# alibaba/pairec

Hardware: AMD Instinct MI355X
Metric: ranked items/sec, 5k-cand DNN rank (recall top-5000 of 100M x 128 -> DNN3 -> fuse -> sort) (higher is better)
Workload: dtype bf16x3; 1 GPU; configs[1]+[2]: recall 5k of 100000000x128 fp32 table in HBM -> 3-layer DNN rank (256-512-256-1, bf16 MFMA with split hi + lo operands = bf16x3, fp32-accurate scores) -> RankScore fusion (fp64) -> ItemRankScore sort; candidates_per_request=5000, table_rows=100000000, dim=128, table_dist=uniform, batches_in_flight=2, contexts=2, all_batches_on_predicted_thresholds=True, batches_re_run_after_a_failed_plan=0, parallelism=1 GPU

## Files before the change

### pairec_amd/csrc/common.hpp

```cpp
#pragma once
#include <hip/hip_runtime.h>

#include <algorithm>
#include <cstdarg>
#include <cstdint>
#include <cstdio>
#include <cstring>
#include <map>
#include <atomic>
#include <memory>
#include <mutex>
#include <shared_mutex>
#include <string>
#include <vector>

#include "../../include/pairec_gpu.h"

namespace pg {

struct PipeRun;
void set_error(const char* fmt, ...);

#define PG_HIP(expr)                                                                           \
    do {                                                                                       \
// ... 404 lines not shown
int rescreen16_prep_launch(pg_ctx* ctx, const pg_table* t, const RecallScratch& rs, uint32_t nq);
int rescreen16_launch(pg_ctx* ctx, const pg_table* t, const RecallScratch& rs, uint32_t nq);
int screen4m_launch(pg_ctx* ctx, const pg_table* t, const RecallScratch& rs, uint32_t nq, uint32_t row_begin, uint32_t row_end,
                    uint32_t cap1, bool susp2_clean = false);
int topk_merge_strided_locked(pg_ctx* ctx, const uint64_t* d_rows, const float* d_scores, uint32_t nq, uint32_t nlists,
                              uint32_t per_list, size_t row_ls, size_t row_qs, size_t sc_ls, size_t sc_qs, uint32_t k,
                              uint64_t* d_out_rows, float* d_out_scores, uint32_t* d_out_count);
int topk_merge_locked(pg_ctx* ctx, const uint64_t* d_rows, const float* d_scores, uint32_t nq, uint32_t nlists,
                      uint32_t per_list, int list_major, uint32_t k, uint64_t* d_out_rows, float* d_out_scores,
                      uint32_t* d_out_count);

int rank_dnn3_dev_locked(pg_ctx* ctx, const pg_model* m, const pg_table* t, const float* d_user,
                         const uint32_t* d_cand, const uint32_t* d_off, uint32_t n_req, uint32_t n_items,
                         float* d_out, size_t out_stride = 0);
int fm2t_user_embedding_locked(pg_ctx* ctx, const pg_model* m, const float* d_user, uint32_t n_req, float* d_out);
int rank_fm2t_irows_dev_locked(pg_ctx* ctx, const pg_model* m, const pg_item_rows* ir, const float* d_user, const int32_t* d_ufids,
                               const uint32_t* d_cand, const uint32_t* d_off, uint32_t n_req, uint32_t n_items, float* d_out);
int rank_fm2t_rows_dev_locked(pg_ctx* ctx, const pg_model* m, const pg_features* fs, const int32_t* item_field_cols,
                              const float* d_user, const int32_t* d_ufids, const uint32_t* d_cand, const uint32_t* d_off,
                              uint32_t n_req, uint32_t n_items, float* d_out);
int expr_eval_enqueue_locked(pg_ctx* ctx, const pg_expr* e, const double* d_vars, uint32_t n_items, double* d_out,
                             uint32_t* d_err, uint32_t items_per_flag);
void set_expr_arith_error(const pg_expr* e);
constexpr int kMaxRewrites = 8;
void expr_hold(const pg_expr* e);
void expr_release(const pg_expr* e);
struct ExprHold {
    const pg_expr* e = nullptr;
    ExprHold() = default;
    ExprHold(const ExprHold&) = delete;
    ExprHold& operator=(const ExprHold&) = delete;
    void take(const pg_expr* x) {
        if (e) expr_release(e);
        e = x;
        if (e) expr_hold(e);
    }
    ~ExprHold() { if (e) expr_release(e); }
};
int expr_num_rewrites(const pg_expr* e);
const char* expr_rewrite_source(const pg_expr* e, int r);
int expr_rewrite_num_vars(const pg_expr* e, int r);
const char* expr_rewrite_var_name(const pg_expr* e, int r, int i);
int expr_rewrite_eval_enqueue_locked(pg_ctx* ctx, const pg_expr* e, int r, const double* d_vars, uint32_t n_items, double* d_out,
                                     uint32_t* d_err, uint32_t items_per_flag);
int table_gather_locked(pg_ctx* ctx, const pg_table* t, const uint32_t* d_rows, uint32_t n, float* d_out);
int dpp_run_locked(pg_ctx* ctx, const float* d_emb32, const double* d_hook, const double* d_rel, uint32_t R, uint32_t n,
// ... 40 lines not shown
```

### pairec_amd/csrc/expr.hip

```cpp
#include "common.hpp"

#include <cmath>
#include <string>
#include <vector>

namespace pg {

enum OpCode : uint32_t { OP_CONST = 0, OP_VAR, OP_ADD, OP_SUB, OP_MUL, OP_DIV, OP_MOD, OP_POW, OP_FNZ,
                         OP_DIVF,
                         OP_NEG };

struct Instr {
    uint32_t op;
    uint32_t arg;
    double val;
};

constexpr int kMaxStack = 32;
constexpr int kMaxProg = 128;

}

struct pg_expr {
    std::string source;
// ... 243 lines not shown
            }
            if (i & 1) {
                a1 *= x1;
                ae += xe;
            }
            x1 *= x1;
            xe <<= 1;
            if (x1 < 0.5) {
                x1 += x1;
                xe--;
            }
        }
        if (y < 0.0) {
            a1 = 1.0 / a1;
            ae = -ae;
        }
        if (ae > 4096) ae = 4096;
        if (ae < -4096) ae = -4096;
        return ldexp(a1, (int)ae);
    }
    return pow(x, y);
}

__global__ void expr_eval_kernel(ExprDev e, const double* __restrict__ vars, uint32_t n_items,
                                 double* __restrict__ out, uint32_t* __restrict__ err, uint32_t items_per_flag) {
    const uint32_t i = blockIdx.x * blockDim.x + threadIdx.x;
    if (i >= n_items) return;
    double st[kMaxStack];
    int sp = 0;
    bool bad = false;
    for (uint32_t pc = 0; pc < e.n; ++pc) {
        const Instr in = e.prog[pc];
        if (in.op == OP_CONST) {
            st[sp++] = in.val;
        } else if (in.op == OP_VAR) {
            st[sp++] = vars[(size_t)in.arg * n_items + i];
        } else {
            if (in.op == OP_NEG) {
                st[sp - 1] = -st[sp - 1];
                continue;
            }
            const double r = st[--sp];
            const double l = st[--sp];
            double v = 0.0;
            switch (in.op) {
                case OP_DIVF: v = l / r; break;
                case OP_ADD: v = l + r; break;
                case OP_SUB: v = l - r; break;
                case OP_MUL: v = l * r; break;
                case OP_DIV:
                    if (r == 0.0) bad = true; else v = l / r;
                    break;
                case OP_MOD: {
                    const long long li = (l == l && fabs(l) < 9223372036854775808.0) ? (long long)l : (long long)0x8000000000000000ull;
                    const long long ri = (r == r && fabs(r) < 9223372036854775808.0) ? (long long)r : (long long)0x8000000000000000ull;
                    if (ri == 0) bad = true;
                    else if (ri == -1) v = 0.0;
                    else v = (double)(li % ri);
                    break;
                }
                case OP_POW: v = go_pow(l, r); break;
                case OP_FNZ: v = (l != 0.0) ? l : r; break;
            }
            st[sp++] = v;
        }
    }
    out[i] = sp > 0 ? st[sp - 1] : 0.0;
    if (bad) atomicOr(err + (items_per_flag ? i / items_per_flag : 0u), 1u);
}

int expr_eval_enqueue_locked(pg_ctx* ctx, const pg_expr* e, const double* d_vars, uint32_t n_items, double* d_out,
                             uint32_t* d_err, uint32_t items_per_flag) {
    if (e->empty) {
        PG_HIP(hipMemsetAsync(d_out, 0, (size_t)n_items * 8, ctx->stream));
    } else {
        ExprDev dev;
        dev.n = (uint32_t)e->prog.size();
        for (size_t i = 0; i < e->prog.size(); ++i) dev.prog[i] = e->prog[i];
        expr_eval_kernel<<<(n_items + 255) / 256, 256, 0, ctx->stream>>>(dev, d_vars, n_items, d_out, d_err, items_per_flag);
        PG_HIP(hipGetLastError());
    }
    return PG_OK;
}

int expr_num_rewrites(const pg_expr* e) { return e ? (int)e->rewrites.size() : 0; }
const char* expr_rewrite_source(const pg_expr* e, int r) { return e->rewrites[(size_t)r].source.c_str(); }
int expr_rewrite_num_vars(const pg_expr* e, int r) { return (int)e->rewrites[(size_t)r].vars.size(); }
const char* expr_rewrite_var_name(const pg_expr* e, int r, int i) { return e->rewrites[(size_t)r].vars[(size_t)i].c_str(); }
int expr_rewrite_eval_enqueue_locked(pg_ctx* ctx, const pg_expr* e, int r, const double* d_vars, uint32_t n_items, double* d_out,
                                     uint32_t* d_err, uint32_t items_per_flag) {
    const pg_expr::Rewrite& rw = e->rewrites[(size_t)r];
    if (rw.failed || rw.prog.empty()) {
        PG_HIP(hipMemsetAsync(d_out, 0, (size_t)n_items * 8, ctx->stream));
        return PG_OK;
    }
    ExprDev dev;
    dev.n = (uint32_t)rw.prog.size();
    for (size_t i = 0; i < rw.prog.size(); ++i) dev.prog[i] = rw.prog[i];
    expr_eval_kernel<<<(n_items + 255) / 256, 256, 0, ctx->stream>>>(dev, d_vars, n_items, d_out, d_err, items_per_flag);
    PG_HIP(hipGetLastError());
    return PG_OK;
}

void set_expr_arith_error(const pg_expr* e) {
    set_error("pg_expr_eval: violation of arithmetic specification: a division by zero in '%s' "
              "(the reference panics in ExprASTResult, utils/ast/ast.go:243-249)", e->source.c_str());
}

static int expr_eval_locked(pg_ctx* ctx, const pg_expr* e, const double* d_vars, uint32_t n_items,
                            double* d_out) {
    void* p;
    int rc;
    if ((rc = scratch_reserve(ctx, 4, 4096, &p))) return rc;
    uint32_t* d_err = (uint32_t*)p + 320;
    PG_HIP(hipMemsetAsync(d_err, 0, 4, ctx->stream));
    if ((rc = expr_eval_enqueue_locked(ctx, e, d_vars, n_items, d_out, d_err, 0))) return rc;
    PG_HIP(hipMemcpyAsync(ctx->h_status + 320, d_err, 4, hipMemcpyDeviceToHost, ctx->stream));
    PG_HIP(hipStreamSynchronize(ctx->stream));
    if (ctx->h_status[320] != 0) {
        set_expr_arith_error(e);
        return PG_ERR_ARITH;
    }
// ... 363 lines not shown
```

### pairec_amd/csrc/misc.hip

```cpp
#include "pipeline.hpp"

#include <algorithm>
#include <cstring>
#include <vector>

namespace pg {

__global__ void rows_to_local_kernel(const uint64_t* __restrict__ rows, uint32_t n, uint64_t off,
                                     uint64_t nrows, uint32_t* __restrict__ local,
                                     uint8_t* __restrict__ owned, uint32_t* __restrict__ uni_off, uint32_t uni_nq, uint32_t uni_k) {
    const uint32_t i = blockIdx.x * blockDim.x + threadIdx.x;
    if (uni_off && i <= uni_nq) uni_off[i] = i * uni_k;
    if (i >= n) return;
    const uint64_t r = rows[i];
    const bool mine = r != ~0ull && r >= off && r - off < nrows;
    local[i] = mine ? (uint32_t)(r - off) : 0u;
    if (owned) owned[i] = mine ? 1 : 0;
}

__global__ void widen_kernel(const float* __restrict__ in, uint32_t n, double* __restrict__ out) {
    const uint32_t i = blockIdx.x * blockDim.x + threadIdx.x;
    if (i < n) out[i] = (double)in[i];
}

typedef uint32_t u32x4 __attribute__((ext_vector_type(4)));
__global__ __launch_bounds__(256) void hbm_probe_kernel(const u32x4* __restrict__ p, uint64_t n16,
                                                        uint32_t* __restrict__ sink) {
    uint32_t acc = 0;
    const uint64_t stride = (uint64_t)gridDim.x * blockDim.x;
    uint64_t i = (uint64_t)blockIdx.x * blockDim.x + threadIdx.x;
    for (; i + 3 * stride < n16; i += 4 * stride) {
        const u32x4 a = __builtin_nontemporal_load(&p[i]);
        const u32x4 b = __builtin_nontemporal_load(&p[i + stride]);
        const u32x4 c = __builtin_nontemporal_load(&p[i + 2 * stride]);
        const u32x4 d = __builtin_nontemporal_load(&p[i + 3 * stride]);
// ... 79 lines not shown
                const uint64_t* d_rows, const float* d_recall, const float* d_rank, size_t rank_stride, int n_algos,
                const double* d_fused, uint32_t nq, uint32_t k, uint32_t top_n, char* d_page) {
    const size_t np = (size_t)nq * top_n;
    if (np == 0) return PG_OK;
    uint64_t* p_rows = (uint64_t*)d_page;
    double* p_fused = (double*)(p_rows + np);
    float* p_recall = (float*)(p_fused + np);
    float* p_rank = p_recall + np;
    page_kernel<<<(uint32_t)((np + 255) / 256), 256, 0, st>>>(d_order, d_pick, d_pick_cnt, d_rows, d_recall, d_rank, rank_stride, n_algos,
                                                             d_fused, nq, k, top_n, p_rows, p_fused, p_recall, p_rank);
    PG_HIP(hipGetLastError());
    return PG_OK;
}

int rows_to_local_locked(pg_ctx* ctx, const pg_table* t, const uint64_t* d_rows, uint32_t n, uint32_t* d_local,
                         uint8_t* d_owned) {
    if (n == 0) return PG_OK;
    rows_to_local_kernel<<<(n + 255) / 256, 256, 0, ctx->stream>>>(d_rows, n, t->row_offset, t->rows, d_local, d_owned, nullptr, 0, 0);
    PG_HIP(hipGetLastError());
    return PG_OK;
}

int rows_to_local_offsets_locked(pg_ctx* ctx, const pg_table* t, const uint64_t* d_rows, uint32_t nq, uint32_t k, uint32_t* d_local,
                                 uint32_t* d_off) {
    const uint32_t n = nq * k;
    if (n <= nq) {
        int rc = uniform_offsets_locked(ctx, nq, k, d_off);
        return rc ? rc : rows_to_local_locked(ctx, t, d_rows, n, d_local, nullptr);
    }
    rows_to_local_kernel<<<(n + 255) / 256, 256, 0, ctx->stream>>>(d_rows, n, t->row_offset, t->rows, d_local, nullptr, d_off, nq, k);
    PG_HIP(hipGetLastError());
    return PG_OK;
}

int uniform_offsets_locked(pg_ctx* ctx, uint32_t nq, uint32_t k, uint32_t* d_off) {
    uniform_offsets_kernel<<<(nq + 256) / 256, 256, 0, ctx->stream>>>(nq, k, d_off);
    PG_HIP(hipGetLastError());
    return PG_OK;
}

}

extern "C" {

int pg_hbm_read_probe(pg_ctx* ctx, const pg_table* t, int reps, double* out_gbps) {
    PG_REQUIRE(ctx && t && out_gbps && reps > 0, "pg_hbm_read_probe: bad argument");
    const void* d_buf = t->d;
    const uint64_t bytes = t->rows * (uint64_t)t->dim * 4;
    PG_REQUIRE(bytes >= (1u << 20), "pg_hbm_read_probe: table smaller than 1 MiB");
    std::lock_guard<std::mutex> g(ctx->mu);
    void* sink;
    int rc;
    if ((rc = pg::scratch_reserve(ctx, 4, 4096, &sink))) return rc;
// ... 37 lines not shown
```

### pairec_amd/csrc/pipeline.hip

```cpp
#include "pipeline.hpp"

#include <algorithm>
#include <chrono>
#include <thread>

namespace pg {

struct VarSrc { int8_t src[32]; };
__global__ void bind_vars_kernel(const float* __restrict__ recall, const float* __restrict__ rank, size_t rank_stride,
                                 uint32_t n, uint32_t nv, VarSrc vs, double* __restrict__ vars, uint32_t* __restrict__ err,
                                 const double* __restrict__ rw, int zero_err) {
    const uint32_t i = blockIdx.x * blockDim.x + threadIdx.x;
    if (zero_err && i < (uint32_t)kMaxQueries) err[i] = 0;
    if (i >= n) return;
    const double a = (double)recall[i];
    for (uint32_t v = 0; v < nv; ++v) {
        const int sa = vs.src[v];
        vars[(size_t)v * n + i] = sa >= 0 ? (double)rank[(size_t)sa * rank_stride + i] : (sa == -1 ? a : rw[(size_t)(-2 - sa) * n + i]);
    }
}

__global__ void mask_pads_kernel(const uint64_t* __restrict__ rows, uint32_t n, float* __restrict__ rank, size_t rank_stride,
                                 int n_algos, double* __restrict__ fused) {
    const uint32_t i = blockIdx.x * blockDim.x + threadIdx.x;
    if (i >= n || rows[i] != ~0ull) return;
    for (int a = 0; a < n_algos; ++a) rank[(size_t)a * rank_stride + i] = 0.0f;
    fused[i] = __longlong_as_double(0x7FF8000000000000ll);
}

int pipe_run_acquire(pg_ctx* ctx, PipeRun** out) {
    {
        std::lock_guard<std::mutex> g(ctx->pool_mu);
        if (!ctx->pipe_free.empty()) {
            *out = ctx->pipe_free.back();
            ctx->pipe_free.pop_back();
            return PG_OK;
        }
    }
    PG_HIP(hipSetDevice(ctx->device));
    PipeRun* r = new PipeRun();
    if (hipHostMalloc((void**)&r->h_status, kPipeStatusWords * 4) != hipSuccess || hipEventCreate(&r->done) != hipSuccess) {
        set_error("pipeline: cannot allocate a batch's status block: %s", hipGetErrorString(hipGetLastError()));
        if (r->h_status) hipHostFree(r->h_status);
// ... 74 lines not shown
    int wide = std::max(c.nv, 1);
    const int n_rw = expr_num_rewrites(c.e);
    for (int r = 0; r < n_rw; ++r) wide = std::max(wide, expr_rewrite_num_vars(c.e, r));
    const size_t b_vars = al((size_t)(wide + n_rw) * n * 8);
    if ((rc = scratch_reserve(ctx, 8, b_local + b_off + b_err + b_vars, &buf))) return rc;
    ps->d_local = (uint32_t*)buf;
    ps->d_off = (uint32_t*)((char*)buf + b_local);
    ps->d_err = (uint32_t*)((char*)buf + b_local + b_off);
    ps->d_vars = (double*)((char*)buf + b_local + b_off + b_err);
    ps->c_rows = nullptr; ps->c_rel = nullptr; ps->c_emb = nullptr; ps->c_bail = nullptr;
    if (c.rerank.kind) {
        const size_t nc = (size_t)nq * c.rerank.candidates;
        const size_t b_rows = al(nc * 8), b_rel = al(nc * 8), b_emb = al(nc * c.t->dim * 4), b_bail = al((size_t)kMaxQueries * 4);
        if ((rc = scratch_reserve(ctx, 10, b_rows + b_rel + b_emb + b_bail, &buf))) return rc;
        ps->c_rows = (uint64_t*)buf;
        ps->c_rel = (double*)((char*)buf + b_rows);
        ps->c_emb = (float*)((char*)buf + b_rows + b_rel);
        ps->c_bail = (uint32_t*)((char*)buf + b_rows + b_rel + b_emb);
    }
    return PG_OK;
}

int fuse_scores_enqueue_locked(pg_ctx* ctx, const pg_expr* e, const int* var_src, int nv, const float* d_recall, const float* d_rank,
                               size_t rank_stride, uint32_t n, uint32_t items_per_flag, double* d_vars, uint32_t* d_err, double* d_fused) {
    hipStream_t st = ctx->stream;
    int rc;
    VarSrc vs;
    const int n_rw = expr_num_rewrites(e);
    int wide = std::max(nv, 1);
    for (int r = 0; r < n_rw; ++r) wide = std::max(wide, expr_rewrite_num_vars(e, r));
    double* const d_rw = d_vars + (size_t)wide * n;
    const uint32_t bind_grid = (std::max(n, (uint32_t)kMaxQueries) + 255) / 256;
    bool zeroed = false;
    for (int r = 0, at = nv; r < n_rw; ++r) {
        const int nvr = expr_rewrite_num_vars(e, r);
        for (int i = 0; i < 32; ++i) vs.src[i] = i < nvr ? (int8_t)var_src[at + i] : (int8_t)-1;
        at += nvr;
        if (nvr > 0 || !zeroed) {
            bind_vars_kernel<<<bind_grid, 256, 0, st>>>(d_recall, d_rank, rank_stride, n, (uint32_t)nvr, vs, d_vars, d_err, nullptr, zeroed ? 0 : 1);
            PG_HIP(hipGetLastError());
            zeroed = true;
        }
        if ((rc = expr_rewrite_eval_enqueue_locked(ctx, e, r, d_vars, n, d_rw + (size_t)r * n, d_err, items_per_flag))) return rc;
    }
    for (int i = 0; i < 32; ++i) vs.src[i] = i < nv ? (int8_t)var_src[i] : (int8_t)-1;
    if (nv > 0) {
        bind_vars_kernel<<<bind_grid, 256, 0, st>>>(d_recall, d_rank, rank_stride, n, (uint32_t)nv, vs, d_vars, d_err, d_rw, zeroed ? 0 : 1);
        PG_HIP(hipGetLastError());
    } else if (!zeroed) {
        PG_HIP(hipMemsetAsync(d_err, 0, (size_t)kMaxQueries * 4, st));
    }
    return expr_eval_enqueue_locked(ctx, e, d_vars, n, d_fused, d_err, items_per_flag);
}

int post_fuse_sort_locked(pg_ctx* ctx, const RecommendCall& c, uint32_t q0, uint32_t nq, const PostScratch& ps) {
    const uint32_t n = nq * c.k;
    const size_t o = (size_t)q0 * c.k;
    hipStream_t st = ctx->stream;
    int rc;
    if ((rc = fuse_scores_enqueue_locked(ctx, c.e, c.var_src, c.nv, c.d_recall + o, c.d_rank + o, c.rank_stride, n, c.k, ps.d_vars, ps.d_err,
                                         c.d_fused + o)))
        return rc;
    if (c.pads) {
        mask_pads_kernel<<<(n + 255) / 256, 256, 0, st>>>(c.d_rows + o, n, c.d_rank + o, c.rank_stride, c.planes(), c.d_fused + o);
        PG_HIP(hipGetLastError());
    }
    return sort_dev_locked(ctx, c.d_fused + o, ps.d_off, nq, n, c.k, 1, c.d_order + o);
}

int rerank_select_locked(pg_ctx* ctx, const RecommendCall& c, uint32_t q0, uint32_t nq, const PostScratch& ps) {
    const uint32_t C = c.rerank.candidates;
    const size_t o = (size_t)q0 * c.k;
    if (c.k < C) {
        set_error("recommend: the DPP stage wants %u candidates, the lists hold k = %u", C, c.k);
        return PG_ERR_UNSUPPORTED;
    }
    int rc;
    if ((rc = sorted_head_launch(ctx->stream, c.d_order + o, c.d_rows + o, c.d_fused + o, nq, c.k, C, ps.c_rows, ps.c_rel))) return rc;
    return dpp_norm_relevance_launch(ctx->stream, ps.c_rel, nq, C, c.rerank.dpp.norm_relevance_score, ps.c_bail);
}
int rerank_run_locked(pg_ctx* ctx, const RecommendCall& c, uint32_t q0, uint32_t nq, const PostScratch& ps) {
    const uint32_t C = c.rerank.candidates;
    int rc;
    if ((rc = dpp_run_locked(ctx, ps.c_emb, nullptr, ps.c_rel, nq, C, c.t->dim, 0, c.rerank.dpp.alpha, c.top_n, c.rerank.dpp.window,
                             c.rerank.dpp.normalize_emb, 1, 1, c.d_pick + (size_t)q0 * c.top_n, c.d_pick_cnt + q0)))
        return rc;
    if (c.rerank.dpp.norm_relevance_score)
        return dpp_bail_fix_launch(ctx->stream, ps.c_bail, nq, C, c.top_n, c.d_pick + (size_t)q0 * c.top_n, c.d_pick_cnt + q0);
    return PG_OK;
}

static int recommend_post_locked(pg_ctx* ctx, const RecommendCall& c, uint32_t q0, uint32_t nq, const PostScratch& ps) {
    const uint32_t n = nq * c.k;
    const size_t o = (size_t)q0 * c.k;
    int rc;
    if ((rc = rows_to_local_offsets_locked(ctx, c.t, c.d_rows + o, nq, c.k, ps.d_local, ps.d_off))) return rc;
    for (int a = 0; a < c.n_algos; ++a) {
        const RankAlgoRef& al = c.algos[a];
        float* out = c.d_rank + (size_t)c.plane0[a] * c.rank_stride + o;
        const float* users = c.d_queries + (size_t)q0 * c.t->dim;
        if ((rc = rank_algo_locked(ctx, al, c.t, users, c.d_ufids ? c.d_ufids + (size_t)q0 * c.ufid_stride : nullptr, ps.d_local, ps.d_off, nq, n,
                                   out, c.rank_stride)))
            return rc;
    }
    if ((rc = post_fuse_sort_locked(ctx, c, q0, nq, ps))) return rc;
    if (c.rerank.kind == 1) {
        if (c.t->rows < c.rerank.candidates) {
            set_error("recommend: the DPP stage wants %u candidates, the table has %llu rows", c.rerank.candidates, (unsigned long long)c.t->rows);
            return PG_ERR_UNSUPPORTED;
        }
        if ((rc = rerank_select_locked(ctx, c, q0, nq, ps))) return rc;
        if ((rc = gather_global_rows_launch(ctx->stream, c.t, ps.c_rows, nq * c.rerank.candidates, ps.c_emb))) return rc;
        if ((rc = rerank_run_locked(ctx, c, q0, nq, ps))) return rc;
    }
    return PG_OK;
}

int rank_algo_locked(pg_ctx* ctx, const RankAlgoRef& al, const pg_table* t, const float* d_user, const int32_t* d_ufids,
                     const uint32_t* d_cand, const uint32_t* d_off, uint32_t n_req, uint32_t n_items, float* d_out, size_t out_stride) {
    if (al.m->kind == PG_MODEL_DNN3) return rank_dnn3_dev_locked(ctx, al.m, t, d_user, d_cand, d_off, n_req, n_items, d_out, out_stride);
    if (al.irows) return rank_fm2t_irows_dev_locked(ctx, al.m, al.irows, d_user, d_ufids, d_cand, d_off, n_req, n_items, d_out);
    return rank_fm2t_rows_dev_locked(ctx, al.m, al.fs, al.item_field_cols, d_user, d_ufids, d_cand, d_off, n_req, n_items, d_out);
}

int recommend_enqueue(pg_ctx* ctx, const RecommendCall& c, PipeRun* r, bool first) {
    if (c.t->d_row_map) {
        set_error("recommend: the table is a filtered view (pg_table_view_create) — views serve the recall calls only");
        return PG_ERR_UNSUPPORTED;
// ... 195 lines not shown
```

### pairec_amd/csrc/pipeline.hpp

```cpp
#pragma once
#include "common.hpp"

namespace pg {

struct RecommendCall;
struct PipeRun {
    RecallJob job;
    uint32_t* h_status = nullptr;
    std::vector<hipEvent_t> events;
    hipEvent_t done = nullptr;
    bool patched = false;
};
constexpr uint32_t kExprFlagAt = 320;
constexpr uint32_t kPipeStatusWords = 640;

int pipe_run_acquire(pg_ctx* ctx, PipeRun** out);
void pipe_run_release(pg_ctx* ctx, PipeRun* r);

constexpr int kMaxAlgos = 4;
struct RankAlgoRef {
    const pg_model* m = nullptr;
    const pg_features* fs = nullptr;
    int32_t item_field_cols[16] = {0};
    const pg_item_rows* irows = nullptr;
// ... 28 lines not shown
    int n_planes = 0;
    int planes() const { return n_planes ? n_planes : n_algos; }
    double* d_fused = nullptr;
    uint32_t* d_order = nullptr;
    uint32_t* d_count = nullptr;
    bool pads = false;
    RerankStage rerank;
    uint32_t top_n = 0;
    uint32_t* d_pick = nullptr;
    uint32_t* d_pick_cnt = nullptr;
};
int recommend_bind_vars(const pg_expr* e, const char* const* names, int n_algos, std::vector<int>* var_src, const char* who);
int recommend_enqueue(pg_ctx* ctx, const RecommendCall& c, PipeRun* r, bool first);
int recommend_verify(pg_ctx* ctx, PipeRun* r, bool* ok, const RecommendCall* c = nullptr);
struct PostScratch {
    uint32_t *d_local, *d_off, *d_err;
    double* d_vars;
    uint64_t* c_rows;
    double* c_rel;
    float* c_emb;
    uint32_t* c_bail;
};
int post_scratch(pg_ctx* ctx, const RecommendCall& c, uint32_t nq, PostScratch* ps);
int post_fuse_sort_locked(pg_ctx* ctx, const RecommendCall& c, uint32_t q0, uint32_t nq, const PostScratch& ps);
int fuse_scores_enqueue_locked(pg_ctx* ctx, const pg_expr* e, const int* var_src, int nv, const float* d_recall, const float* d_rank,
                               size_t rank_stride, uint32_t n, uint32_t items_per_flag, double* d_vars, uint32_t* d_err, double* d_fused);
int rerank_select_locked(pg_ctx* ctx, const RecommendCall& c, uint32_t q0, uint32_t nq, const PostScratch& ps);
int rerank_run_locked(pg_ctx* ctx, const RecommendCall& c, uint32_t q0, uint32_t nq, const PostScratch& ps);

int rows_to_local_locked(pg_ctx* ctx, const pg_table* t, const uint64_t* d_rows, uint32_t n, uint32_t* d_local,
                         uint8_t* d_owned);
int uniform_offsets_locked(pg_ctx* ctx, uint32_t nq, uint32_t k, uint32_t* d_off);
int rows_to_local_offsets_locked(pg_ctx* ctx, const pg_table* t, const uint64_t* d_rows, uint32_t nq, uint32_t k, uint32_t* d_local,
                                 uint32_t* d_off);
int sorted_head_launch(hipStream_t st, const uint32_t* d_order, const uint64_t* d_rows, const double* d_fused, uint32_t nq,
                       uint32_t k, uint32_t C, uint64_t* d_c_rows, double* d_c_rel);
int gather_global_rows_launch(hipStream_t st, const pg_table* t, const uint64_t* d_global_rows, uint32_t n, float* d_out);
size_t page_entry_bytes(int n_algos);
int page_launch(hipStream_t st, const uint32_t* d_order, const uint32_t* d_pick, const uint32_t* d_pick_cnt,
                const uint64_t* d_rows, const float* d_recall, const float* d_rank, size_t rank_stride, int n_algos,
                const double* d_fused, uint32_t nq, uint32_t k, uint32_t top_n, char* d_page);
int dpp_norm_relevance_launch(hipStream_t st, double* d_rel, uint32_t nq, uint32_t n, int mode, uint32_t* d_bail);
int dpp_bail_fix_launch(hipStream_t st, const uint32_t* d_bail, uint32_t nq, uint32_t n, uint32_t top_n, uint32_t* d_pick,
                        uint32_t* d_pick_cnt);
bool dpp_norm_relevance_host(const double* rel, uint32_t n, int mode, double* out);
int ssd_run_locked(pg_ctx* ctx, const pg_table* t, const uint32_t* d_cand, const double* d_rel, uint32_t R, uint32_t n,
                   double gamma, uint32_t T, uint32_t window, int normalize_emb, int ensure_pos_similarity, int use_ssd_star,
                   uint32_t* d_out);
bool ssd_batchable(uint32_t d1, uint32_t window);
bool ssd_norm_quality_host(const double* rel, uint32_t n, int mode, double* out);

}
```

### pairec_amd/csrc/recall.hip

```cpp
#include "common.hpp"
#include "bitonic_reg.hpp"
#include "split_sort.hpp"

#include <type_traits>

namespace pg {

typedef float f32x16 __attribute__((ext_vector_type(16)));
typedef float f32x4 __attribute__((ext_vector_type(4)));

constexpr int kPieceRows = 32;
constexpr int kPieceCols = 32;
constexpr int kPieceBytes = kPieceRows * kPieceCols * 4;
constexpr int kPieceDmas = kPieceBytes / 1024;
constexpr int kPieceQuads = kPieceCols / 4;
constexpr int kRingSlots = 4;
constexpr int kScanWaves = 8;
constexpr int kScanLdsRing = kScanWaves * kRingSlots * kPieceBytes;
constexpr int kStageCap = 280;
constexpr int kStageBytes = kStageCap * 12 + 512;
constexpr int kScanLds = kScanLdsRing + kScanWaves * kStageBytes;

__device__ __forceinline__ uint32_t f32_ordered_bits(float f) {
    const uint32_t b = __float_as_uint(f);
// ... 853 lines not shown
        s = __fmaf_rn(x.x, y.x, s);
        s = __fmaf_rn(x.y, y.y, s);
        s = __fmaf_rn(x.z, y.z, s);
        s = __fmaf_rn(x.w, y.w, s);
        if ((k & 3) == 3) __builtin_amdgcn_sched_barrier(0);
    }
    __builtin_amdgcn_wave_barrier();
}

template <int DIM, bool L2 = false>
__global__ __launch_bounds__(256) void rescore_kernel(const float* __restrict__ tab, const float* __restrict__ qpad,
                                                      const float* __restrict__ thr,
                                                      const uint32_t* __restrict__ susp,
                                                      const uint32_t* __restrict__ susp_cnt, uint32_t cap,
                                                      uint32_t* __restrict__ cnt, uint64_t* __restrict__ cand,
                                                      uint32_t* __restrict__ overflow, uint32_t scap, uint32_t n_rows,
                                                      const float* __restrict__ nx = nullptr, const float* __restrict__ nqv = nullptr,
                                                      RowFilter filter = RowFilter()) {
    constexpr int kRowB = 64 * 4 + 16;
    __shared__ __attribute__((aligned(16))) char tile[4][64 * kRowB];
    __shared__ __attribute__((aligned(16))) float qs[DIM];
    __shared__ uint32_t wsum[4];
    __shared__ uint32_t base_s;
    const uint32_t q = blockIdx.y;
    const uint32_t n_raw = susp_cnt[q];
    const uint32_t n = n_raw < scap ? n_raw : scap;
    if (blockIdx.x * 256u >= n) return;
    const int lane = threadIdx.x & 63, w = threadIdx.x >> 6;
    if (threadIdx.x < DIM) qs[threadIdx.x] = qpad[(size_t)q * DIM + threadIdx.x];
    const float thr_q = thr[q];
    __syncthreads();
    char* const my = tile[w];
    auto row_of = [&](uint32_t t0) -> uint32_t {
        const uint32_t e = t0 + threadIdx.x;
        const uint32_t r = e < n ? susp[(uint64_t)q * scap + e] : 0u;
        return r < n_rows ? r : 0u;
    };
    constexpr int NPH = DIM / 64;
    const uint32_t step = gridDim.x * 256u;
    uint32_t t0 = blockIdx.x * 256u;
    uint32_t row = row_of(t0);
    f32x4 va[16], vb[16];
    rescore_gather<DIM>(va, tab, row, 0, lane);
    for (; t0 < n; t0 += step) {
        const bool valid = t0 + threadIdx.x < n;
        const uint32_t row_next = t0 + step < n ? row_of(t0 + step) : 0u;
        float s = 0.0f;
        if constexpr (NPH == 1) {
            rescore_gather<DIM>(vb, tab, row_next, 0, lane);
            rescore_walk<kRowB>(va, my, qs, 0, lane, s);
        } else if constexpr (NPH == 2) {
            rescore_gather<DIM>(vb, tab, row, 1, lane);
            rescore_walk<kRowB>(va, my, qs, 0, lane, s);
            rescore_gather<DIM>(va, tab, row_next, 0, lane);
            rescore_walk<kRowB>(vb, my, qs, 1, lane, s);
        } else if constexpr (NPH == 3) {
            rescore_gather<DIM>(vb, tab, row, 1, lane);
            rescore_walk<kRowB>(va, my, qs, 0, lane, s);
            rescore_gather<DIM>(va, tab, row, 2, lane);
            rescore_walk<kRowB>(vb, my, qs, 1, lane, s);
            rescore_gather<DIM>(vb, tab, row_next, 0, lane);
            rescore_walk<kRowB>(va, my, qs, 2, lane, s);
        } else {
            static_assert(NPH == 4, "rescore_kernel: DIM 64, 128, 192 or 256");
            rescore_gather<DIM>(vb, tab, row, 1, lane);
            rescore_walk<kRowB>(va, my, qs, 0, lane, s);
            rescore_gather<DIM>(va, tab, row, 2, lane);
            rescore_walk<kRowB>(vb, my, qs, 1, lane, s);
            rescore_gather<DIM>(vb, tab, row, 3, lane);
// ... 2 lines not shown
            rescore_walk<kRowB>(vb, my, qs, 3, lane, s);
        }
        if (NPH & 1) {
#pragma unroll
            for (int i = 0; i < 16; ++i) va[i] = vb[i];
        }
        if constexpr (L2) s = __fmaf_rn(2.0f, s, -(nx[row] + nqv[q]));
        const bool keep = valid && !(s < thr_q) && row_filter_pass(filter, row);
        const uint64_t m = __builtin_amdgcn_ballot_w64(keep);
        const uint32_t before = __builtin_amdgcn_mbcnt_hi((uint32_t)(m >> 32), __builtin_amdgcn_mbcnt_lo((uint32_t)m, 0u));
        if (lane == 0) wsum[w] = __popcll(m);
        __syncthreads();
        if (threadIdx.x == 0) {
            const uint32_t tot = wsum[0] + wsum[1] + wsum[2] + wsum[3];
            base_s = tot ? atomicAdd(&cnt[q], tot) : 0u;
        }
        __syncthreads();
        uint32_t pos = base_s + before;
        for (int j = 0; j < w; ++j) pos += wsum[j];
        if (keep) {
            if (pos < cap) cand[(uint64_t)q * cap + pos] = topk_key(s, row);
            else *overflow = 1u;
        }
        __syncthreads();
        row = row_next;
    }
    if (n_raw > scap && threadIdx.x == 0) *overflow = 1u;
}

__global__ void screen_prep_kernel(const float* __restrict__ qpad, uint32_t dim,
                                   uint4* __restrict__ qb16, float* __restrict__ eps) {
    const uint32_t KS = dim / 16;
    const uint32_t i = blockIdx.x * blockDim.x + threadIdx.x;
    if (i < (uint32_t)kScreenMaxNQB * KS * 64) {
        const uint32_t lane = i & 63, ks = (i >> 6) % KS, c = (i >> 6) / KS;
        const float* q = qpad + (size_t)(c * 32 + (lane & 31)) * dim + ks * 16 + 8 * (lane >> 5);
        uint32_t w[4];
        for (int e = 0; e < 4; ++e) {
            auto rne = [](float x) -> uint32_t {
                uint32_t b = __float_as_uint(x);
                if ((b & 0x7FFFFFFFu) > 0x7F800000u) return (b >> 16) | 0x40u;
                b += 0x7FFFu + ((b >> 16) & 1u);
                return b >> 16;
            };
            w[e] = rne(q[2 * e]) | (rne(q[2 * e + 1]) << 16);
        }
        qb16[i] = make_uint4(w[0], w[1], w[2], w[3]);
    }
    if (i < (uint32_t)kMaxQueries) {
        double ss = 0.0;
// ... 749 lines not shown
    if (a.nx) {
        if (dim == 64) return wide ? launch_scan<64, 2, true>(ctx, a) : launch_scan<64, 1, true>(ctx, a);
        if (dim == 128) return wide ? launch_scan<128, 2, true>(ctx, a) : launch_scan<128, 1, true>(ctx, a);
        set_error("recall (squared Euclidean): dim=%u unsupported (64 or 128)", dim);
        return PG_ERR_UNSUPPORTED;
    }
    switch (dim) {
        case 64: return wide ? launch_scan<64, 2>(ctx, a) : launch_scan<64, 1>(ctx, a);
        case 128: return wide ? launch_scan<128, 2>(ctx, a) : launch_scan<128, 1>(ctx, a);
        case 192:
        case 256:
            if (wide) {
                set_error("recall: dim=%u supports at most 32 queries per pass (64 up to dim 128)", dim);
                return PG_ERR_UNSUPPORTED;
            }
            return dim == 192 ? launch_scan<192, 1>(ctx, a) : launch_scan<256, 1>(ctx, a);
    }
    set_error("recall: dim=%u unsupported", dim);
    return PG_ERR_UNSUPPORTED;
}

constexpr uint32_t kFirstChunkRows = 32768;
constexpr uint32_t kRescoreBlocksPerQuery = 16;
constexpr uint32_t kCandSlack = 1u << 19;

int recall_scratch(pg_ctx* ctx, uint32_t dim, uint32_t k, RecallScratch* rs) {
    const uint32_t cap = k + kCandSlack;
    void* small;
    int rc;
    const size_t qb16_bytes = (size_t)kScreenMaxNQB * (dim / 16) * 64 * 16;
    const size_t small_bytes = (size_t)kMaxQueries * dim * 4 + qb16_bytes + (size_t)kMaxQueries * 40 + 2048 + (size_t)kQ4mWords * 4 + 256 + 64 +
                               (size_t)kMaxQueries * (2 * 128 + 16 + 4) + 192 + (size_t)(kRecallStatusWords + kMaxQueries) * 4 + 64;
    if ((rc = scratch_reserve(ctx, 2, small_bytes, &small))) return rc;
    rs->qpad = (float*)small;
    rs->qb16 = (uint4*)((char*)small + (size_t)kMaxQueries * dim * 4);
    rs->thr = (float*)((char*)rs->qb16 + qb16_bytes);
    rs->eps = rs->thr + kMaxQueries;
    rs->thr_screen = rs->eps + kMaxQueries;
    rs->cnt = (uint32_t*)(rs->thr_screen + kMaxQueries);
    rs->susp_cnt = rs->cnt + kMaxQueries;
    rs->overflow = rs->susp_cnt + kMaxQueries;
    rs->qscale = (float*)(rs->overflow + 64 + kMaxQueries);
    rs->q4 = (uint32_t*)(rs->qscale + kMaxQueries);
    rs->thr_ref = (float*)(rs->q4 + 160);
    rs->pred_ms = rs->thr_ref + kMaxQueries;
    rs->susp2_cnt = (uint32_t*)(rs->pred_ms + 2 * kMaxQueries);
// ... 692 lines not shown
            const uint32_t scap = i4 ? rs.cap * (uint32_t)(kMaxQueries / kI4MaxQueries) : rs.cap;
            const uint64_t r_begin = (uint64_t)rb * kPieceRows;
            const uint64_t r_end = (uint64_t)(rb + cb) * kPieceRows < j->rows ? (uint64_t)(rb + cb) * kPieceRows : j->rows;
            if (i4) {
                if ((rc2 = screen4_launch(ctx, t, rs, nq, (uint32_t)r_begin, (uint32_t)r_end, scap, j->l2 ? rs.pred_ms : nullptr))) return rc2;
                j->scan_bytes += (r_end - r_begin) * (j->l2 ? 72 : 68);
            } else if (i4m) {
                if ((rc2 = screen4m_launch(ctx, t, rs, nq, (uint32_t)r_begin, (uint32_t)r_end, rs.cap * (uint32_t)(kMaxQueries / kI4mMaxQueries), susp2_clean))) return rc2;
                susp2_clean = false;
                j->scan_bytes += (r_end - r_begin) * 68;
                last_was_i4m = true;
            } else {
                last_was_i4m = false;
                if ((rc2 = dispatch_screen(ctx, t->dim, t->shadow_is_i8, sa))) return rc2;
                if (records) {
                    screen_decode_kernel<<<rec_waves / 8 + sa.rec_pool_cap / kRecPoolSlice, 1024, 0, ctx->stream>>>(
                        sa.rec, sa.rec_cnt, sa.rec_cap, rec_waves, sa.rec_pool, sa.rec_pool_cap, rs.thr_screen, j->rows,
                                                                            rs.susp_cnt, rs.susp, rs.cap, rs.overflow);
                    PG_HIP(hipGetLastError());
                }
                j->scan_bytes += (uint64_t)cb * kPieceRows * t->dim * (t->shadow_is_i8 ? 1 : 2);
            }
            j->scanned_rows += (uint64_t)cb * kPieceRows;
            const dim3 rg(i4 ? screen4_rescore_blocks() : kRescoreBlocksPerQuery, nq);
            const bool r2 = j->stage2 && t->shadow_is_i8 && !i4 && !i4m && !j->l2 && t->dim == 128;
            if (r2) {
                if ((rc2 = rescreen16_launch(ctx, t, rs, nq))) return rc2;
                last_was_r2 = true;
                rescore_kernel<128><<<rg, 256, 0, ctx->stream>>>(t->d, rs.qpad, rs.thr, rs.susp2, rs.susp2w_cnt, rs.cap,
                                                                 rs.cnt, rs.cand[cur], rs.overflow, rs.cap, j->rows, nullptr, nullptr, j->filter);
            } else if (j->l2)
                rescore_kernel<128, true><<<rg, 256, 0, ctx->stream>>>(t->d, rs.qpad, rs.thr, rs.susp, rs.susp_cnt, rs.cap, rs.cnt,
                                                                       rs.cand[cur], rs.overflow, scap, j->rows, t->d_nx, rs.pred_ms, j->filter);
            else if (t->dim == 64)
                rescore_kernel<64><<<rg, 256, 0, ctx->stream>>>(t->d, rs.qpad, rs.thr, rs.susp, rs.susp_cnt, rs.cap,
                                                                rs.cnt, rs.cand[cur], rs.overflow, scap, j->rows, nullptr, nullptr, j->filter);
            else if (i4m)
                rescore_kernel<128><<<rg, 256, 0, ctx->stream>>>(t->d, rs.qpad, rs.thr, rs.susp2, rs.susp2_cnt, rs.cap,
                                                                 rs.cnt, rs.cand[cur], rs.overflow, rs.cap, j->rows, nullptr, nullptr, j->filter);
            else
                rescore_kernel<128><<<rg, 256, 0, ctx->stream>>>(t->d, rs.qpad, rs.thr, rs.susp, rs.susp_cnt, rs.cap,
                                                                 rs.cnt, rs.cand[cur], rs.overflow, scap, j->rows, nullptr, nullptr, j->filter);
            PG_HIP(hipGetLastError());
        } else {
            last_full_screened = false;
            ScanArgs a;
            a.tab = t->d;
// ... 769 lines not shown
```

Baseline: 278.1 million ranked items/s.

## Fuse variable binding into expr eval, fold err zeroing, balance rescore blocks

Replaces the separate bind_vars kernel with an expression evaluator that reads recall, rank and rewrite values straight from their sources. This removes one kernel launch and the staging writes to the vars buffer. Zeroing of the error flags moves into the rows_to_local kernel, so the memset disappears too. The rescore kernel is also reworked: each block computes a prefix sum of per-query suspect counts and takes an even slice of the combined 256-row tiles, and the grid is sized from the CU count instead of a fixed 16 blocks per query. The rescore change aims to balance load across queries with skewed suspect counts, at the cost of extra prefix-sum work and query-switch logic in every block.

New measurement: 278.5 million ranked items/s, median of 3. About the same (+0.1%).

```diff
diff --git a/pairec_amd/csrc/common.hpp b/pairec_amd/csrc/common.hpp
--- a/pairec_amd/csrc/common.hpp
+++ b/pairec_amd/csrc/common.hpp
@@ -450,6 +450,15 @@
 int expr_eval_enqueue_locked(pg_ctx* ctx, const pg_expr* e, const double* d_vars, uint32_t n_items, double* d_out,
                              uint32_t* d_err, uint32_t items_per_flag);
 void set_expr_arith_error(const pg_expr* e);
+struct ExprSrc {
+    const float* recall;
+    const float* rank;
+    size_t rank_stride;
+    const double* rw;
+    int8_t src[32];
+};
+int expr_eval_src_enqueue_locked(pg_ctx* ctx, const pg_expr* e, int r, const ExprSrc& src, uint32_t n_items, double* d_out,
+                                 uint32_t* d_err, uint32_t items_per_flag);
 constexpr int kMaxRewrites = 8;
 void expr_hold(const pg_expr* e);
 void expr_release(const pg_expr* e);
diff --git a/pairec_amd/csrc/expr.hip b/pairec_amd/csrc/expr.hip
--- a/pairec_amd/csrc/expr.hip
+++ b/pairec_amd/csrc/expr.hip
@@ -289,19 +289,16 @@
     return pow(x, y);
 }
 
-__global__ void expr_eval_kernel(ExprDev e, const double* __restrict__ vars, uint32_t n_items,
-                                 double* __restrict__ out, uint32_t* __restrict__ err, uint32_t items_per_flag) {
-    const uint32_t i = blockIdx.x * blockDim.x + threadIdx.x;
-    if (i >= n_items) return;
+template <class Load>
+__device__ __forceinline__ double expr_run(const ExprDev& e, Load load, bool& bad) {
     double st[kMaxStack];
     int sp = 0;
-    bool bad = false;
     for (uint32_t pc = 0; pc < e.n; ++pc) {
         const Instr in = e.prog[pc];
         if (in.op == OP_CONST) {
             st[sp++] = in.val;
         } else if (in.op == OP_VAR) {
-            st[sp++] = vars[(size_t)in.arg * n_items + i];
+            st[sp++] = load(in.arg);
         } else {
             if (in.op == OP_NEG) {
                 st[sp - 1] = -st[sp - 1];
@@ -332,7 +329,27 @@
             st[sp++] = v;
         }
     }
-    out[i] = sp > 0 ? st[sp - 1] : 0.0;
+    return sp > 0 ? st[sp - 1] : 0.0;
+}
+
+__global__ void expr_eval_kernel(ExprDev e, const double* __restrict__ vars, uint32_t n_items,
+                                 double* __restrict__ out, uint32_t* __restrict__ err, uint32_t items_per_flag) {
+    const uint32_t i = blockIdx.x * blockDim.x + threadIdx.x;
+    if (i >= n_items) return;
+    bool bad = false;
+    out[i] = expr_run(e, [&](uint32_t v) { return vars[(size_t)v * n_items + i]; }, bad);
+    if (bad) atomicOr(err + (items_per_flag ? i / items_per_flag : 0u), 1u);
+}
+
+__global__ void expr_eval_src_kernel(ExprDev e, ExprSrc s, uint32_t n_items, double* __restrict__ out, uint32_t* __restrict__ err,
+                                     uint32_t items_per_flag) {
+    const uint32_t i = blockIdx.x * blockDim.x + threadIdx.x;
+    if (i >= n_items) return;
+    bool bad = false;
+    out[i] = expr_run(e, [&](uint32_t v) {
+        const int sa = s.src[v];
+        return sa >= 0 ? (double)s.rank[(size_t)sa * s.rank_stride + i] : (sa == -1 ? (double)s.recall[i] : s.rw[(size_t)(-2 - sa) * n_items + i]);
+    }, bad);
     if (bad) atomicOr(err + (items_per_flag ? i / items_per_flag : 0u), 1u);
 }
 
@@ -365,6 +382,27 @@
     dev.n = (uint32_t)rw.prog.size();
     for (size_t i = 0; i < rw.prog.size(); ++i) dev.prog[i] = rw.prog[i];
     expr_eval_kernel<<<(n_items + 255) / 256, 256, 0, ctx->stream>>>(dev, d_vars, n_items, d_out, d_err, items_per_flag);
+    PG_HIP(hipGetLastError());
+    return PG_OK;
+}
+
+int expr_eval_src_enqueue_locked(pg_ctx* ctx, const pg_expr* e, int r, const ExprSrc& src, uint32_t n_items, double* d_out,
+                                 uint32_t* d_err, uint32_t items_per_flag) {
+    const std::vector<Instr>* prog = &e->prog;
+    if (r >= 0) {
+        const pg_expr::Rewrite& rw = e->rewrites[(size_t)r];
+        prog = rw.failed ? nullptr : &rw.prog;
+    } else if (e->empty) {
+        prog = nullptr;
+    }
+    if (!prog || (r >= 0 && prog->empty())) {
+        PG_HIP(hipMemsetAsync(d_out, 0, (size_t)n_items * 8, ctx->stream));
+        return PG_OK;
+    }
+    ExprDev dev;
+    dev.n = (uint32_t)prog->size();
+    for (size_t i = 0; i < prog->size(); ++i) dev.prog[i] = (*prog)[i];
+    expr_eval_src_kernel<<<(n_items + 255) / 256, 256, 0, ctx->stream>>>(dev, src, n_items, d_out, d_err, items_per_flag);
     PG_HIP(hipGetLastError());
     return PG_OK;
 }
diff --git a/pairec_amd/csrc/misc.hip b/pairec_amd/csrc/misc.hip
--- a/pairec_amd/csrc/misc.hip
+++ b/pairec_amd/csrc/misc.hip
@@ -8,9 +8,11 @@
 
 __global__ void rows_to_local_kernel(const uint64_t* __restrict__ rows, uint32_t n, uint64_t off,
                                      uint64_t nrows, uint32_t* __restrict__ local,
-                                     uint8_t* __restrict__ owned, uint32_t* __restrict__ uni_off, uint32_t uni_nq, uint32_t uni_k) {
+                                     uint8_t* __restrict__ owned, uint32_t* __restrict__ uni_off, uint32_t uni_nq, uint32_t uni_k,
+                                     uint32_t* __restrict__ zero = nullptr, uint32_t n_zero = 0) {
     const uint32_t i = blockIdx.x * blockDim.x + threadIdx.x;
     if (uni_off && i <= uni_nq) uni_off[i] = i * uni_k;
+    if (i < n_zero) zero[i] = 0u;
     if (i >= n) return;
     const uint64_t r = rows[i];
     const bool mine = r != ~0ull && r >= off && r - off < nrows;
@@ -136,13 +138,16 @@
 }
 
 int rows_to_local_offsets_locked(pg_ctx* ctx, const pg_table* t, const uint64_t* d_rows, uint32_t nq, uint32_t k, uint32_t* d_local,
-                                 uint32_t* d_off) {
+                                 uint32_t* d_off, uint32_t* d_zero, uint32_t n_zero) {
     const uint32_t n = nq * k;
+    if (!d_zero) n_zero = 0;
     if (n <= nq) {
+        if (n_zero) PG_HIP(hipMemsetAsync(d_zero, 0, (size_t)n_zero * 4, ctx->stream));
         int rc = uniform_offsets_locked(ctx, nq, k, d_off);
         return rc ? rc : rows_to_local_locked(ctx, t, d_rows, n, d_local, nullptr);
     }
-    rows_to_local_kernel<<<(n + 255) / 256, 256, 0, ctx->stream>>>(d_rows, n, t->row_offset, t->rows, d_local, nullptr, d_off, nq, k);
+    rows_to_local_kernel<<<(std::max(n, n_zero) + 255) / 256, 256, 0, ctx->stream>>>(d_rows, n, t->row_offset, t->rows, d_local, nullptr, d_off, nq, k,
+                                                                                    d_zero, n_zero);
     PG_HIP(hipGetLastError());
     return PG_OK;
 }
diff --git a/pairec_amd/csrc/pipeline.hip b/pairec_amd/csrc/pipeline.hip
--- a/pairec_amd/csrc/pipeline.hip
+++ b/pairec_amd/csrc/pipeline.hip
@@ -5,20 +5,6 @@
 #include <thread>
 
 namespace pg {
-
-struct VarSrc { int8_t src[32]; };
-__global__ void bind_vars_kernel(const float* __restrict__ recall, const float* __restrict__ rank, size_t rank_stride,
-                                 uint32_t n, uint32_t nv, VarSrc vs, double* __restrict__ vars, uint32_t* __restrict__ err,
-                                 const double* __restrict__ rw, int zero_err) {
-    const uint32_t i = blockIdx.x * blockDim.x + threadIdx.x;
-    if (zero_err && i < (uint32_t)kMaxQueries) err[i] = 0;
-    if (i >= n) return;
-    const double a = (double)recall[i];
-    for (uint32_t v = 0; v < nv; ++v) {
-        const int sa = vs.src[v];
-        vars[(size_t)v * n + i] = sa >= 0 ? (double)rank[(size_t)sa * rank_stride + i] : (sa == -1 ? a : rw[(size_t)(-2 - sa) * n + i]);
-    }
-}
 
 __global__ void mask_pads_kernel(const uint64_t* __restrict__ rows, uint32_t n, float* __restrict__ rank, size_t rank_stride,
                                  int n_algos, double* __restrict__ fused) {
@@ -139,44 +125,37 @@
 }
 
 int fuse_scores_enqueue_locked(pg_ctx* ctx, const pg_expr* e, const int* var_src, int nv, const float* d_recall, const float* d_rank,
-                               size_t rank_stride, uint32_t n, uint32_t items_per_flag, double* d_vars, uint32_t* d_err, double* d_fused) {
-    hipStream_t st = ctx->stream;
-    int rc;
-    VarSrc vs;
+                               size_t rank_stride, uint32_t n, uint32_t items_per_flag, double* d_vars, uint32_t* d_err, double* d_fused,
+                               bool err_zeroed) {
+    int rc;
+    ExprSrc es;
+    es.recall = d_recall;
+    es.rank = d_rank;
+    es.rank_stride = rank_stride;
+    es.rw = nullptr;
     const int n_rw = expr_num_rewrites(e);
     int wide = std::max(nv, 1);
     for (int r = 0; r < n_rw; ++r) wide = std::max(wide, expr_rewrite_num_vars(e, r));
     double* const d_rw = d_vars + (size_t)wide * n;
-    const uint32_t bind_grid = (std::max(n, (uint32_t)kMaxQueries) + 255) / 256;
-    bool zeroed = false;
+    if (!err_zeroed) PG_HIP(hipMemsetAsync(d_err, 0, (size_t)kMaxQueries * 4, ctx->stream));
     for (int r = 0, at = nv; r < n_rw; ++r) {
         const int nvr = expr_rewrite_num_vars(e, r);
-        for (int i = 0; i < 32; ++i) vs.src[i] = i < nvr ? (int8_t)var_src[at + i] : (int8_t)-1;
+        for (int i = 0; i < 32; ++i) es.src[i] = i < nvr ? (int8_t)var_src[at + i] : (int8_t)-1;
         at += nvr;
-        if (nvr > 0 || !zeroed) {
-            bind_vars_kernel<<<bind_grid, 256, 0, st>>>(d_recall, d_rank, rank_stride, n, (uint32_t)nvr, vs, d_vars, d_err, nullptr, zeroed ? 0 : 1);
-            PG_HIP(hipGetLastError());
-            zeroed = true;
-        }
-        if ((rc = expr_rewrite_eval_enqueue_locked(ctx, e, r, d_vars, n, d_rw + (size_t)r * n, d_err, items_per_flag))) return rc;
-    }
-    for (int i = 0; i < 32; ++i) vs.src[i] = i < nv ? (int8_t)var_src[i] : (int8_t)-1;
-    if (nv > 0) {
-        bind_vars_kernel<<<bind_grid, 256, 0, st>>>(d_recall, d_rank, rank_stride, n, (uint32_t)nv, vs, d_vars, d_err, d_rw, zeroed ? 0 : 1);
-        PG_HIP(hipGetLastError());
-    } else if (!zeroed) {
-        PG_HIP(hipMemsetAsync(d_err, 0, (size_t)kMaxQueries * 4, st));
-    }
-    return expr_eval_enqueue_locked(ctx, e, d_vars, n, d_fused, d_err, items_per_flag);
-}
-
-int post_fuse_sort_locked(pg_ctx* ctx, const RecommendCall& c, uint32_t q0, uint32_t nq, const PostScratch& ps) {
+        if ((rc = expr_eval_src_enqueue_locked(ctx, e, r, es, n, d_rw + (size_t)r * n, d_err, items_per_flag))) return rc;
+    }
+    for (int i = 0; i < 32; ++i) es.src[i] = i < nv ? (int8_t)var_src[i] : (int8_t)-1;
+    es.rw = d_rw;
+    return expr_eval_src_enqueue_locked(ctx, e, -1, es, n, d_fused, d_err, items_per_flag);
+}
+
+int post_fuse_sort_locked(pg_ctx* ctx, const RecommendCall& c, uint32_t q0, uint32_t nq, const PostScratch& ps, bool err_zeroed) {
     const uint32_t n = nq * c.k;
     const size_t o = (size_t)q0 * c.k;
     hipStream_t st = ctx->stream;
     int rc;
     if ((rc = fuse_scores_enqueue_locked(ctx, c.e, c.var_src, c.nv, c.d_recall + o, c.d_rank + o, c.rank_stride, n, c.k, ps.d_vars, ps.d_err,
-                                         c.d_fused + o)))
+                                         c.d_fused + o, err_zeroed)))
         return rc;
     if (c.pads) {
         mask_pads_kernel<<<(n + 255) / 256, 256, 0, st>>>(c.d_rows + o, n, c.d_rank + o, c.rank_stride, c.planes(), c.d_fused + o);
@@ -211,7 +190,7 @@
     const uint32_t n = nq * c.k;
     const size_t o = (size_t)q0 * c.k;
     int rc;
-    if ((rc = rows_to_local_offsets_locked(ctx, c.t, c.d_rows + o, nq, c.k, ps.d_local, ps.d_off))) return rc;
+    if ((rc = rows_to_local_offsets_locked(ctx, c.t, c.d_rows + o, nq, c.k, ps.d_local, ps.d_off, ps.d_err, (uint32_t)kMaxQueries))) return rc;
     for (int a = 0; a < c.n_algos; ++a) {
         const RankAlgoRef& al = c.algos[a];
         float* out = c.d_rank + (size_t)c.plane0[a] * c.rank_stride + o;
@@ -220,7 +199,7 @@
                                    out, c.rank_stride)))
             return rc;
     }
-    if ((rc = post_fuse_sort_locked(ctx, c, q0, nq, ps))) return rc;
+    if ((rc = post_fuse_sort_locked(ctx, c, q0, nq, ps, true))) return rc;
     if (c.rerank.kind == 1) {
         if (c.t->rows < c.rerank.candidates) {
             set_error("recommend: the DPP stage wants %u candidates, the table has %llu rows", c.rerank.candidates, (unsigned long long)c.t->rows);
diff --git a/pairec_amd/csrc/pipeline.hpp b/pairec_amd/csrc/pipeline.hpp
--- a/pairec_amd/csrc/pipeline.hpp
+++ b/pairec_amd/csrc/pipeline.hpp
@@ -74,9 +74,10 @@
     uint32_t* c_bail;
 };
 int post_scratch(pg_ctx* ctx, const RecommendCall& c, uint32_t nq, PostScratch* ps);
-int post_fuse_sort_locked(pg_ctx* ctx, const RecommendCall& c, uint32_t q0, uint32_t nq, const PostScratch& ps);
+int post_fuse_sort_locked(pg_ctx* ctx, const RecommendCall& c, uint32_t q0, uint32_t nq, const PostScratch& ps, bool err_zeroed = false);
 int fuse_scores_enqueue_locked(pg_ctx* ctx, const pg_expr* e, const int* var_src, int nv, const float* d_recall, const float* d_rank,
-                               size_t rank_stride, uint32_t n, uint32_t items_per_flag, double* d_vars, uint32_t* d_err, double* d_fused);
+                               size_t rank_stride, uint32_t n, uint32_t items_per_flag, double* d_vars, uint32_t* d_err, double* d_fused,
+                               bool err_zeroed = false);
 int rerank_select_locked(pg_ctx* ctx, const RecommendCall& c, uint32_t q0, uint32_t nq, const PostScratch& ps);
 int rerank_run_locked(pg_ctx* ctx, const RecommendCall& c, uint32_t q0, uint32_t nq, const PostScratch& ps);
 
@@ -84,7 +85,7 @@
                          uint8_t* d_owned);
 int uniform_offsets_locked(pg_ctx* ctx, uint32_t nq, uint32_t k, uint32_t* d_off);
 int rows_to_local_offsets_locked(pg_ctx* ctx, const pg_table* t, const uint64_t* d_rows, uint32_t nq, uint32_t k, uint32_t* d_local,
-                                 uint32_t* d_off);
+                                 uint32_t* d_off, uint32_t* d_zero = nullptr, uint32_t n_zero = 0);
 int sorted_head_launch(hipStream_t st, const uint32_t* d_order, const uint64_t* d_rows, const double* d_fused, uint32_t nq,
                        uint32_t k, uint32_t C, uint64_t* d_c_rows, double* d_c_rel);
 int gather_global_rows_launch(hipStream_t st, const pg_table* t, const uint64_t* d_global_rows, uint32_t n, float* d_out);
diff --git a/pairec_amd/csrc/recall.hip b/pairec_amd/csrc/recall.hip
--- a/pairec_amd/csrc/recall.hip
+++ b/pairec_amd/csrc/recall.hip
@@ -899,29 +899,61 @@
     __shared__ __attribute__((aligned(16))) float qs[DIM];
     __shared__ uint32_t wsum[4];
     __shared__ uint32_t base_s;
-    const uint32_t q = blockIdx.y;
-    const uint32_t n_raw = susp_cnt[q];
-    const uint32_t n = n_raw < scap ? n_raw : scap;
-    if (blockIdx.x * 256u >= n) return;
+    __shared__ uint32_t pre[kMaxQueries + 1];
+    __shared__ uint32_t nlist[kMaxQueries];
+    static_assert(kMaxQueries <= 256, "rescore_kernel: one thread per query list");
     const int lane = threadIdx.x & 63, w = threadIdx.x >> 6;
+    const uint32_t nq = gridDim.y;
+    {
+        const uint32_t n_raw = threadIdx.x < nq ? susp_cnt[threadIdx.x] : 0u;
+        const uint32_t n = n_raw < scap ? n_raw : scap;
+        if (n_raw > scap && blockIdx.x == 0 && blockIdx.y == 0) *overflow = 1u;
+        uint32_t c = (n + 255u) >> 8;
+#pragma unroll
+        for (int d = 1; d < 64; d <<= 1) {
+            const uint32_t o = (uint32_t)__shfl_up((int)c, d, 64);
+            if (lane >= d) c += o;
+        }
+        if (lane == 63) wsum[w] = c;
+        if (threadIdx.x < (uint32_t)kMaxQueries) nlist[threadIdx.x] = n;
+        __syncthreads();
+        for (int jw = 0; jw < w; ++jw) c += wsum[jw];
+        if (threadIdx.x < (uint32_t)kMaxQueries) pre[threadIdx.x + 1] = c;
+        if (threadIdx.x == 0) pre[0] = 0u;
+        __syncthreads();
+    }
+    const uint32_t total = pre[nq];
+    const uint32_t nblk = gridDim.x * gridDim.y, blk = blockIdx.y * gridDim.x + blockIdx.x;
+    uint32_t it = (uint32_t)((uint64_t)blk * total / nblk);
+    const uint32_t it_end = (uint32_t)((uint64_t)(blk + 1) * total / nblk);
+    if (it >= it_end) return;
+    uint32_t q = 0;
+    while (it >= pre[q + 1]) ++q;
     if (threadIdx.x < DIM) qs[threadIdx.x] = qpad[(size_t)q * DIM + threadIdx.x];
-    const float thr_q = thr[q];
+    float thr_q = thr[q];
     __syncthreads();
     char* const my = tile[w];
-    auto row_of = [&](uint32_t t0) -> uint32_t {
+    auto row_of = [&](uint32_t qq, uint32_t t0) -> uint32_t {
         const uint32_t e = t0 + threadIdx.x;
-        const uint32_t r = e < n ? susp[(uint64_t)q * scap + e] : 0u;
+        const uint32_t r = e < nlist[qq] ? susp[(uint64_t)qq * scap + e] : 0u;
         return r < n_rows ? r : 0u;
     };
     constexpr int NPH = DIM / 64;
-    const uint32_t step = gridDim.x * 256u;
-    uint32_t t0 = blockIdx.x * 256u;
-    uint32_t row = row_of(t0);
+    uint32_t row = row_of(q, (it - pre[q]) * 256u);
     f32x4 va[16], vb[16];
     rescore_gather<DIM>(va, tab, row, 0, lane);
-    for (; t0 < n; t0 += step) {
-        const bool valid = t0 + threadIdx.x < n;
-        const uint32_t row_next = t0 + step < n ? row_of(t0 + step) : 0u;
+    for (; it < it_end; ++it) {
+        const bool valid = (it - pre[q]) * 256u + threadIdx.x < nlist[q];
+        const bool more = it + 1 < it_end;
+        uint32_t q_next = q;
+        if (more)
+            while (it + 1 >= pre[q_next + 1]) ++q_next;
+        const uint32_t row_next = more ? row_of(q_next, (it + 1 - pre[q_next]) * 256u) : 0u;
+        float qv_next = 0.0f, thr_next = thr_q;
+        if (q_next != q) {
+            if (threadIdx.x < DIM) qv_next = qpad[(size_t)q_next * DIM + threadIdx.x];
+            thr_next = thr[q_next];
+        }
         float s = 0.0f;
         if constexpr (NPH == 1) {
             rescore_gather<DIM>(vb, tab, row_next, 0, lane);
@@ -970,10 +1002,14 @@
             if (pos < cap) cand[(uint64_t)q * cap + pos] = topk_key(s, row);
             else *overflow = 1u;
         }
+        if (q_next != q) {
+            if (threadIdx.x < DIM) qs[threadIdx.x] = qv_next;
+            thr_q = thr_next;
+            q = q_next;
+        }
         __syncthreads();
         row = row_next;
     }
-    if (n_raw > scap && threadIdx.x == 0) *overflow = 1u;
 }
 
 __global__ void screen_prep_kernel(const float* __restrict__ qpad, uint32_t dim,
@@ -1769,6 +1805,11 @@
 
 constexpr uint32_t kFirstChunkRows = 32768;
 constexpr uint32_t kRescoreBlocksPerQuery = 16;
+constexpr uint32_t kRescoreBlocksPerCU = 2;
+static uint32_t rescore_blocks(const pg_ctx* ctx, uint32_t nq) {
+    const uint32_t x = (kRescoreBlocksPerCU * (uint32_t)ctx->num_cus + nq - 1) / nq;
+    return x < 1 ? 1u : (x > kRescoreBlocksPerQuery ? kRescoreBlocksPerQuery : x);
+}
 constexpr uint32_t kCandSlack = 1u << 19;
 
 int recall_scratch(pg_ctx* ctx, uint32_t dim, uint32_t k, RecallScratch* rs) {
@@ -2507,7 +2548,7 @@
                 j->scan_bytes += (uint64_t)cb * kPieceRows * t->dim * (t->shadow_is_i8 ? 1 : 2);
             }
             j->scanned_rows += (uint64_t)cb * kPieceRows;
-            const dim3 rg(i4 ? screen4_rescore_blocks() : kRescoreBlocksPerQuery, nq);
+            const dim3 rg(i4 ? screen4_rescore_blocks() : rescore_blocks(ctx, nq), nq);
             const bool r2 = j->stage2 && t->shadow_is_i8 && !i4 && !i4m && !j->l2 && t->dim == 128;
             if (r2) {
                 if ((rc2 = rescreen16_launch(ctx, t, rs, nq))) return rc2;
```
